# weigert/SoilMachine

Measured on AMD Instinct MI355X. Metric: particle-steps/s, higher is better.
Workload: dtype f64

## Files before the change

include/soilmx.h:

```cpp
#ifndef SOILMX_H
#define SOILMX_H
#include <stdint.h>

#ifdef __cplusplus
extern "C" {
#endif

typedef struct smx_ctx smx_ctx;

typedef struct smx_soil {
  uint32_t transports, erodes, cascades, abrades;
  float density, porosity, solubility, equrate, friction, erosionrate, maxdiff, settling, suspension, abrasion;
} smx_soil;

typedef struct smx_layer {
  uint32_t type;
  float min, bias, scale, octaves, lacunarity, gain, frequency;
} smx_layer;

enum { SMX_ENGINE_SERIAL = 0,
       SMX_ENGINE_SPECULATIVE = 1,
       SMX_ENGINE_BATCHED = 2,
       SMX_ENGINE_RELAXED = 3       };

// ... 159 lines not shown
int smx_fill_vertex_cut(smx_ctx* ctx, const float* colors4, int32_t ncolors, int32_t mode, double cut, int32_t x, int32_t y, void* out_vertex44);
int smx_heights_bilinear(smx_ctx* ctx, const float* pos2, int32_t n, double* out);

int smx_digest(smx_ctx* ctx, double* sumh, uint64_t* nsec, uint64_t* typehash);
int smx_switches(char* buf, uint64_t cap, uint64_t* needed);
int smx_get_counters_sized(smx_ctx* ctx, smx_counters* out, uint64_t struct_size);
int smx_get_timing_sized(smx_ctx* ctx, smx_timing* out, uint64_t struct_size);
int smx_get_counters(smx_ctx* ctx, smx_counters* out);
int smx_get_timing(smx_ctx* ctx, smx_timing* out);
int smx_timing_reset(smx_ctx* ctx);
int smx_set_engine(smx_ctx* ctx, int32_t engine);
int smx_set_spec_limits(smx_ctx* ctx, uint32_t particles_per_subphase, uint32_t nested_slots);
int smx_set_batch_dilate(smx_ctx* ctx, int32_t tiles);
int smx_set_relax_wind(smx_ctx* ctx, uint32_t min_running, int32_t steps_per_epoch);
int smx_set_relax_launch(smx_ctx* ctx, int32_t persistent, int32_t tail_at);
int smx_set_grid_interleave(smx_ctx* ctx, int32_t k);
int smx_set_water_generations(smx_ctx* ctx, int32_t k);
int smx_get_water_generations(smx_ctx* ctx, int32_t* k);
int smx_set_water_stagger(smx_ctx* ctx, int32_t gap_epochs);
int smx_get_water_stagger(smx_ctx* ctx, int32_t* gap_epochs);
int smx_set_batch_strips(smx_ctx* ctx, int32_t nstrips, int32_t inset, int32_t seam_halfwidth);
int smx_d_set_own(smx_ctx* ctx, int32_t own_x0, int32_t own_x1);
int smx_d_gen_begin(smx_ctx* ctx, int32_t wind, uint32_t nslots, const void* children, uint32_t* contains_out);
int smx_d_gen_spawn(smx_ctx* ctx, const uint32_t* contains, uint32_t* nlive_local);
int smx_d_next_phase(smx_ctx* ctx);
int smx_d_chunk(smx_ctx* ctx, uint32_t nlive_global, uint32_t* nlive_local);
int smx_d_gen_end(smx_ctx* ctx, void* children_out, uint32_t cap, uint32_t* n);
int smx_d_pack_columns(smx_ctx* ctx, int32_t x0, int32_t x1, void* buf, uint64_t cap, uint64_t* bytes);
int smx_d_unpack_columns(smx_ctx* ctx, const void* buf, uint64_t bytes);
int smx_d_pack_particles(smx_ctx* ctx, int32_t x0, int32_t x1, void* buf, uint64_t cap, uint64_t* bytes);
// ... 41 lines not shown
```

soilmachine_amd/capi.py:

```python
from __future__ import annotations

import ctypes as C
import os

import numpy as np

_HERE = os.path.dirname(os.path.abspath(__file__))
LIB_PATH = os.path.join(_HERE, "libsoilmx.so")

ENGINE_SERIAL = 0
ENGINE_SPECULATIVE = 1
ENGINE_BATCHED = 2
ENGINE_RELAXED = 3


class Config(C.Structure):
    _fields_ = [("dimx", C.c_int32), ("dimy", C.c_int32), ("scale", C.c_int32), ("device", C.c_int32),
                ("pool_capacity", C.c_uint64), ("engine", C.c_int32), ("reserved", C.c_int32)]


class Counters(C.Structure):
    _fields_ = [(n, C.c_uint64) for n in (
        "steps_water_top", "steps_water_all", "steps_wind", "nested_particles", "floods", "cascade_calls",
        "cascade_transfers", "wcascade_calls", "grid_active_cells", "rand_calls", "pool_free", "pool_overflow",
# ... 85 lines not shown
LAKE_DRY = 0xFFFFFFFF
LAKE_BORDER, LAKE_VOLUME_UNRELIABLE = 1, 2
DRAIN_NONE = 0xFFFFFFFF
BASIN_LAKE, BASIN_BORDER = 1, 2

PLANE_HEIGHT, PLANE_WATER, PLANE_WFREQ, PLANE_WINDFREQ = 0, 1, 2, 3
PLANES = {"height": PLANE_HEIGHT, "water": PLANE_WATER, "wfreq": PLANE_WFREQ, "windfreq": PLANE_WINDFREQ}


SYMBOLS = [
    "smx_create", "smx_create_strip", "smx_destroy", "smx_last_error", "smx_set_soils", "smx_set_scale", "smx_srand", "smx_rand", "smx_rand_advance", "smx_get_rand_state", "smx_set_rand_state",
    "smx_initialize", "smx_import_columns", "smx_import_frequency", "smx_num_sections", "smx_export_columns",
    "smx_read_frequency", "smx_read_heights", "smx_read_surface", "smx_tick_water", "smx_grid_pass", "smx_tick_wind",
    "smx_map_frequency", "smx_reset_frequency", "smx_tick", "smx_sync", "smx_add", "smx_remove",
    "smx_particle_cascade", "smx_water_cascade", "smx_seep", "smx_top", "smx_normals", "smx_heights_bilinear", "smx_fill_vertices", "smx_fill_vertices_cut", "smx_fill_vertex_cut",
    "smx_digest", "smx_save", "smx_load", "smx_get_counters", "smx_get_timing", "smx_get_counters_sized", "smx_get_timing_sized", "smx_timing_reset", "smx_set_engine", "smx_set_spec_limits", "smx_stream", "smx_set_batch_dilate", "smx_get_batch_stats", "smx_set_batch_strips", "smx_set_relax_wind", "smx_set_relax_launch", "smx_set_grid_interleave", "smx_set_water_generations", "smx_get_water_generations", "smx_set_water_stagger", "smx_get_water_stagger", "smx_strips_rccl_unique_id", "smx_strips_attach_rccl", "smx_strips_attach", "smx_strips_detach", "smx_strips_tick", "smx_strips_stats", "smx_strips_sync_stats", "smx_strips_selfcheck",
    "smx_d_set_own", "smx_d_gen_begin", "smx_d_gen_spawn", "smx_d_next_phase", "smx_d_chunk", "smx_d_gen_end", "smx_d_pack_columns",
    "smx_d_unpack_columns", "smx_d_pack_particles", "smx_d_unpack_particles", "smx_d_grid_begin", "smx_d_grid_sweep_cols",
    "smx_lbm_create", "smx_lbm_destroy", "smx_lbm_last_error", "smx_lbm_set_boundary", "smx_lbm_boundary_from_map", "smx_lbm_initialize",
    "smx_lbm_step", "smx_lbm_read", "smx_lbm_write_f", "smx_lbm_move", "smx_lbm_get_timing",
    "smx_ensemble_create", "smx_ensemble_destroy", "smx_ensemble_last_error", "smx_ensemble_add", "smx_ensemble_remove", "smx_ensemble_size",
    "smx_ensemble_tick", "smx_ensemble_sync", "smx_ensemble_get_timing", "smx_ensemble_timing_reset",
    "smx_ensemble_figures", "smx_ensemble_plane_stats", "smx_copy_state", "smx_ensemble_fork",
    "smx_lakes", "smx_ensemble_lakes", "smx_drainage", "smx_ensemble_drainage",
    "smx_soil_totals", "smx_ensemble_soil_totals", "smx_soil_thickness", "smx_cores",
    "smx_switches",
]

ENSEMBLE_MAX_MEMBERS = 4096

_lib = None
# ... 50 lines not shown
    L.smx_get_counters.argtypes = [vp, C.POINTER(Counters)]
    L.smx_get_timing.argtypes = [vp, C.POINTER(Timing)]
    L.smx_get_counters_sized.argtypes = [vp, C.POINTER(Counters), u64]
    L.smx_get_timing_sized.argtypes = [vp, C.POINTER(Timing), u64]
    L.smx_timing_reset.argtypes = [vp]
    L.smx_set_engine.argtypes = [vp, i32]
    L.smx_set_water_generations.argtypes = [vp, i32]
    L.smx_get_water_generations.argtypes = [vp, C.POINTER(i32)]
    L.smx_set_water_stagger.argtypes = [vp, i32]
    L.smx_get_water_stagger.argtypes = [vp, C.POINTER(i32)]
    L.smx_set_spec_limits.argtypes = [vp, C.c_uint32, C.c_uint32]
    L.smx_set_batch_dilate.argtypes = [vp, i32]
    L.smx_set_batch_strips.argtypes = [vp, i32, i32, i32]
    L.smx_set_relax_wind.argtypes = [vp, u32, i32]
    L.smx_set_relax_launch.argtypes = [vp, i32, i32]
    L.smx_create_strip.argtypes = [C.POINTER(Config), i32, i32, C.POINTER(vp)]
    L.smx_strips_rccl_unique_id.argtypes = [vp]
    L.smx_strips_attach_rccl.argtypes = [vp, vp, i32, i32, i32, i32]
    L.smx_strips_attach.argtypes = [vp, C.POINTER(Transport), i32, i32, i32, i32]
    L.smx_strips_detach.argtypes = [vp]
    L.smx_strips_tick.argtypes = [vp, i32, i32, i32, i32]
    L.smx_strips_stats.argtypes = [vp] + [C.POINTER(u64)] * 5
    L.smx_strips_sync_stats.argtypes = [vp] + [C.POINTER(u64)] * 2
    L.smx_strips_selfcheck.argtypes = [vp, u32, u32, u32]
    L.smx_d_set_own.argtypes = [vp, i32, i32]
    L.smx_d_gen_begin.argtypes = [vp, i32, u32, vp, vp]
    L.smx_d_gen_spawn.argtypes = [vp, vp, C.POINTER(u32)]
    L.smx_d_next_phase.argtypes = [vp]
    L.smx_d_chunk.argtypes = [vp, u32, C.POINTER(u32)]
    L.smx_d_gen_end.argtypes = [vp, vp, u32, C.POINTER(u32)]
# ... 70 lines not shown
```

soilmachine_amd/csrc/soil_relax.h:

```cpp
#pragma once
#include "soil_batch.h"

namespace smx {

constexpr uint32_t R_TRACK = 1, R_ERODE = 2, R_DEPOSIT = 4, R_WINDFREQ = 8, R_LIFT = 16;

#ifdef SMX_HOSTSIM
SMX_D uint32_t relax_append(uint32_t* counter, bool want) { return want ? SMX_A_ADD(counter, 1u) : NIL; }
#else
SMX_D uint32_t relax_append(uint32_t* counter, bool want) {
  const unsigned long long m = __ballot(want);
  if (!want) return NIL;
  const int leader = __ffsll((long long)m) - 1, lane = (int)(threadIdx.x & 63u);
  uint32_t base = 0u;
  if (lane == leader) base = atomicAdd(counter, (uint32_t)__popcll(m));
  base = (uint32_t)__shfl((int)base, leader);
  return base + (uint32_t)__popcll(m & ((1ull << lane) - 1ull));
}
#endif
SMX_D uint32_t relax_colour(const DevState& s, uint32_t c) {
  const uint32_t x = c / (uint32_t)s.dimy, y = c - x * (uint32_t)s.dimy;
  return (x % 3u) * 3u + (y % 3u);
}
SMX_D void relax_push(const DevState& s, const BatchShared& bs, uint32_t e, const RReq& r, uint32_t epoch) {
// ... 5 lines not shown
  if (flag) { if (k < bs.flag_cap) bs.flagl[par][k] = r.casc; else SMX_A_ADD(&bs.ctrl[BC_LIST_LOST], 1u); }
  (void)s;
}
SMX_D void relax_flood_later(const BatchShared& bs, uint32_t slot, uint32_t parity, bool want = true) {
  const uint32_t k = relax_append(&bs.ctrl[BC_NFLOOD + parity], want);
  if (want) { if (k < bs.list_cap) bs.flist[parity][k] = slot; else SMX_A_ADD(&bs.ctrl[BC_LIST_LOST], 1u); }
}
SMX_D void relax_reset_lists(const BatchShared& bs, uint32_t par) {
  bs.ctrl[BC_NFLOOD + par] = 0u; bs.ctrl[BC_NFLAG + par] = 0u; bs.ctrl[BC_NRUN + par] = 0u;
  for (uint32_t q = 0; q < 9u; q++) bs.ctrl[BC_NCASC + 9u * par + q] = 0u;
}
constexpr unsigned long long RELAX_FLOOD_SHARE = 64ull;
SMX_D bool relax_floods_due(const BatchShared& bs, uint32_t epoch, uint32_t nflood, uint32_t nrun) {
  return bs.strips.n > 1 || (epoch & 3u) == 3u || (unsigned long long)nflood * RELAX_FLOOD_SHARE >= (unsigned long long)nrun;
}
template <class P>
SMX_D void relax_filter(Sim<P>& sim, const BatchShared& bs, uint32_t c, bool valid, uint32_t epoch) {
  const DevState& s = sim.s;
  bool need = false; uint32_t col = 0u;
  if (valid) {
    const int x = (int)(c / (uint32_t)s.dimy), y = (int)(c - (uint32_t)x * (uint32_t)s.dimy);
    Blk b;
    sim.template load_block<2>(x, y, b);
    need = sim.cascade_precheck(b);
    if (!need) sim.n_casc++;
    else {
      bool alone = true;
      const int xa = x - 2 < s.x_lo ? s.x_lo : x - 2, xb = x + 2 >= s.x_hi ? s.x_hi - 1 : x + 2;
      const int ya = y - 2 < 0 ? 0 : y - 2, yb = y + 2 >= s.dimy ? s.dimy - 1 : y + 2;
      for (int xx = xa; xx <= xb; xx++)
        for (int yy = ya; yy <= yb; yy++)
          if ((xx != x || yy != y) && bs.cflag[(size_t)xx * (size_t)s.dimy + (size_t)yy] == bs.rtag) alone = false;
      if (alone) { sim.cascade_blk(x, y, b); need = false; }
    }
    col = (uint32_t)((x % 3) * 3 + (y % 3));
  }
  const uint32_t par = epoch & 1u;
#pragma unroll 1
  for (uint32_t q = 0; q < 9u; q++) {
    const bool mine = need && col == q;
    const uint32_t k = relax_append(&bs.ctrl[BC_NCASC + 9u * par + q], mine);
    if (mine) { if (k < bs.clist_cap) bs.clist[par][(size_t)q * bs.clist_cap + k] = c; else SMX_A_ADD(&bs.ctrl[BC_LIST_LOST], 1u); }
    if (mine && k < bs.clist_cap && bs.cstate) bs.cstate[c] = 2u * bs.rtag;
  }
}

template <class P>
// ... 177 lines not shown
```

soilmachine_amd/csrc/soilmx.hip:

```cpp
#include <hip/hip_runtime.h>
#include <stdint.h>
#include <stdio.h>
#include <string.h>
#include <stdlib.h>
#include <sys/stat.h>
#include <dlfcn.h>
#include <string>
#include <vector>

#include "../../include/soilmx.h"
#ifdef SMX_PROF_FLOOD
__device__ unsigned long long g_sect[32];
#endif
#include "soil_core.h"
#include "soil_serial.h"
#include "soil_spec.h"
#include <type_traits>
#include <chrono>
#include "soil_coop.h"
#include "soil_noise.h"
#include "soil_batch.h"
#include "soil_relax.h"
#include "soil_devmem.h"
#include "soil_lbm.h"
// ... 498 lines not shown
  }
  if (i >= nlive) return;
  BatchPolicy pol(s, bs);
  Sim<BatchPolicy> sim(s, sh, pol);
  relax_apply_slot(sim, bs, bs.live[i]);
  sim.flush_counters(); pol.finish(s);
}
__device__ __forceinline__ void relax_commit_cascade_counters(const DevState& s, unsigned long long nc, unsigned long long nt) {
  for (int off = 32; off > 0; off >>= 1) { nc += (unsigned long long)__shfl_down((long long)nc, off); nt += (unsigned long long)__shfl_down((long long)nt, off); }
  if ((threadIdx.x & 63u) == 0) { if (nc) atomicAdd(&s.ctr[C_CASCADE_CALLS], nc); if (nt) atomicAdd(&s.ctr[C_CASCADE_TRANSFERS], nt); }
}
__device__ __forceinline__ void relax_commit_flood_steps(const DevState& s, unsigned long long n) {
  for (int off = 32; off > 0; off >>= 1) n += (unsigned long long)__shfl_down((long long)n, off);
  if ((threadIdx.x & 63u) == 0 && n) atomicAdd(&s.ctr[C_FLOOD_NESTED_STEPS], n);
}
__global__ void __launch_bounds__(64) k_relax_filter(DevState s, BatchShared bs, uint32_t epoch) {
  const uint32_t par = epoch & 1u;
  uint32_t n = bs.ctrl[BC_NFLAG + par];
  if (n > bs.flag_cap) n = bs.flag_cap;
  if (blockIdx.x * 64u >= n) return;
  SMX_LOAD_SOILS(sh)
  const uint32_t i = blockIdx.x * 64u + threadIdx.x;
  BatchPolicy pol(s, bs);
  Sim<BatchPolicy> sim(s, sh, pol);
  relax_filter(sim, bs, i < n ? bs.flagl[par][i] : 0u, i < n, epoch);
  sim.flush_counters(); pol.finish(s);
  relax_commit_cascade_counters(s, pol.a_casc, pol.a_tr);
}
__global__ void __launch_bounds__(64) k_relax_cascade(DevState s, BatchShared bs, uint32_t epoch, uint32_t colour) {
  const uint32_t par = epoch & 1u;
  uint32_t n = bs.ctrl[BC_NCASC + 9u * par + colour];
  if (n > bs.clist_cap) n = bs.clist_cap;
  if (blockIdx.x * 64u >= n) return;
  SMX_LOAD_SOILS(sh)
  unsigned long long nc = 0, nt = 0;
  for (uint32_t i = blockIdx.x * 64u + threadIdx.x; i < n; i += gridDim.x * 64u) {
    BatchPolicy pol(s, bs);
    Sim<BatchPolicy> sim(s, sh, pol);
    relax_cascade(sim, bs.clist[par][(size_t)colour * bs.clist_cap + i]);
    sim.flush_counters(); pol.finish(s);
    nc += pol.a_casc; nt += pol.a_tr;
  }
  relax_commit_cascade_counters(s, nc, nt);
}
static uint32_t spin_budget(uint32_t dflt) { static const long long v = env_int("SMX_SPIN_BUDGET"); return v >= 0 ? (uint32_t)v : dflt; }
__device__ __forceinline__ bool spin_wait_while(const uint32_t* f, uint32_t busy, uint32_t* stalled, uint32_t budget, uint32_t sleep_a, uint32_t naps) {
  uint32_t spins = 0;
  while (__hip_atomic_load(f, __ATOMIC_RELAXED, __HIP_MEMORY_SCOPE_AGENT) == busy) {
    if (sleep_a == 2u) __builtin_amdgcn_s_sleep(2); else __builtin_amdgcn_s_sleep(8);
    for (uint32_t r = 0; r < naps; r++) __builtin_amdgcn_s_sleep(127);
    if (++spins > budget) { __hip_atomic_store(stalled, 1u, __ATOMIC_RELAXED, __HIP_MEMORY_SCOPE_AGENT); return false; }
    if ((spins & 1023u) == 0u && __hip_atomic_load(stalled, __ATOMIC_RELAXED, __HIP_MEMORY_SCOPE_AGENT)) return false;
  }
  return true;
}
__global__ void __launch_bounds__(64) k_relax_cascade_flow(DevState s, BatchShared bs, uint32_t epoch, uint32_t budget) {
  const uint32_t par = epoch & 1u;
  uint32_t cnt[9], total = 0;
#pragma unroll
  for (uint32_t q = 0; q < 9u; q++) { uint32_t n = bs.ctrl[BC_NCASC + 9u * par + q]; if (n > bs.clist_cap) n = bs.clist_cap; cnt[q] = n; total += n; }
  if (total == 0u) return;
  SMX_LOAD_SOILS(sh)
  __shared__ uint32_t s_i;
  unsigned long long nc = 0, nt = 0;
  const uint32_t pending = 2u * bs.rtag;
  bool live = true;
  while (true) {
    if (threadIdx.x == 0) s_i = atomicAdd(&bs.ctrl[BC_CASC_CURSOR], 1u);
    __syncthreads();
    uint32_t i = s_i;
    __syncthreads();
    if (i >= total) break;
    if (threadIdx.x == 0) {
      uint32_t q = 0;
#pragma unroll
      for (uint32_t k = 0; k < 9u; k++) { if (q == k && i >= cnt[k]) { i -= cnt[k]; q = k + 1u; } }
      const uint32_t c = bs.clist[par][(size_t)q * bs.clist_cap + i];
      const int x = (int)(c / (uint32_t)s.dimy), y = (int)(c - (uint32_t)x * (uint32_t)s.dimy);
      const int xa = x - 2 < s.x_lo ? s.x_lo : x - 2, xb = x + 2 >= s.x_hi ? s.x_hi - 1 : x + 2;
      const int ya = y - 2 < 0 ? 0 : y - 2, yb = y + 2 >= s.dimy ? s.dimy - 1 : y + 2;
      for (int xx = xa; xx <= xb; xx++)
        for (int yy = ya; yy <= yb; yy++) {
          if ((uint32_t)((xx % 3) * 3 + (yy % 3)) >= q) continue;
          uint32_t* f = &bs.cstate[(size_t)xx * (size_t)s.dimy + (size_t)yy];
          if (live && !spin_wait_while(f, pending, &bs.ctrl[BC_STALLED], budget, 2u, 0u)) live = false;
        }
      __atomic_thread_fence(__ATOMIC_ACQUIRE);
      BatchPolicy pol(s, bs);
      Sim<BatchPolicy> sim(s, sh, pol);
      relax_cascade(sim, c);
      sim.flush_counters(); pol.finish(s);
      nc += pol.a_casc; nt += pol.a_tr;
      __hip_atomic_store(&bs.cstate[c], pending + 1u, __ATOMIC_RELEASE, __HIP_MEMORY_SCOPE_AGENT);
    }
  }
  if (threadIdx.x == 0) { if (nc) atomicAdd(&s.ctr[C_CASCADE_CALLS], nc); if (nt) atomicAdd(&s.ctr[C_CASCADE_TRANSFERS], nt); }
}
__device__ unsigned long long g_flood_prof[72];
__global__ void __launch_bounds__(64) k_relax_floods(DevState s, BatchShared bs, uint32_t epoch, uint32_t prof) {
  const uint32_t par = epoch & 1u;
  uint32_t n = bs.ctrl[BC_NFLOOD + par];
  if (n > bs.list_cap) n = bs.list_cap;
  uint32_t lpw = (n + gridDim.x - 1u) / gridDim.x;
  if (lpw > 64u) lpw = 64u;
  if (blockIdx.x * lpw >= n) return;
  SMX_LOAD_SOILS(sh)
  const uint32_t i = blockIdx.x * lpw + threadIdx.x;
  const bool act = threadIdx.x < lpw && i < n;
  bool again = false; uint32_t slot = 0u;
  if (!relax_floods_due(bs, epoch, n, bs.ctrl[BC_NRUN + par])) {
    if (act) slot = bs.flist[par][i];
// ... 777 lines not shown
  bool batch_wind_buf = false;
  uint32_t* d_draws = nullptr; uint32_t* h_draws = nullptr; uint32_t draws_cap = 0;
  BChild* d_kids = nullptr; uint32_t kids_cap = 0;
  unsigned long long* d_skeys[2] = {nullptr, nullptr}; uint32_t* d_sidx[2] = {nullptr, nullptr}; void* d_stemp = nullptr; size_t stemp_bytes = 0; uint32_t sort_cap = 0;
  uint32_t* h_bctrl = nullptr;
  int batch_dilate = 0;
  uint32_t relax_wind_min = 0xFFFFFFFFu;
  int relax_wind_steps = 4;
  int relax_water_steps = 1;
  uint32_t relax_tag = 0;
  struct GridBar* d_gbar = nullptr;
  int mega_blocks = 0;
  bool mega_off = false;
  int relax_persistent = -1, relax_tail_at = -1;
  uint32_t flood_launch_no = 0;
  uint32_t relax_cap = 0;
  int strips_n = 1, strips_a = 16, strips_b = 48;
  int own_x0 = 0, own_x1 = -1;
  bool d_wind = false, d_first = true; uint32_t d_nslots = 0, d_epoch = 0, d_chunk = 0;
  uint32_t* d_contains = nullptr; uint32_t contains_cap = 0;
  uint8_t* d_xdata = nullptr; uint32_t* d_xoffs = nullptr; XCursor* d_xcur = nullptr;
  unsigned long long xdata_cap = 0; uint32_t xoffs_cap = 0;
  uint8_t* d_rdata = nullptr; uint32_t* d_roffs = nullptr; uint8_t* d_xpart = nullptr; uint8_t* d_rpart = nullptr; unsigned long long xpart_cap = 0;
  struct StripState* strip = nullptr;
  uint32_t* d_tdone = nullptr; uint32_t* d_tpend[2] = {nullptr, nullptr}; uint32_t* d_tcount = nullptr; uint32_t* h_tcount = nullptr; void* d_tsort = nullptr; size_t tsort_bytes = 0; uint32_t tsort_cap = 0;
  uint64_t batch_epochs = 0, batch_generations = 0, batch_children_lost = 0, grid_passes = 0;
  ForkScratch fork;
  LakeScratch lakes;
  DrainScratch drain;
  StrataScratch strata;
// ... 222 lines not shown
int smx_get_water_stagger(smx_ctx* ctx, int32_t* gap_epochs) { if (!gap_epochs) return -2; *gap_epochs = ctx->water_stagger; return 0; }
int smx_set_water_generations(smx_ctx* ctx, int32_t k) {
  if (k < 1 || k > 64) { ctx->err = "smx_set_water_generations: 1..64"; return -2; }
  ctx->water_generations = k;
  return 0;
}
int smx_set_grid_interleave(smx_ctx* ctx, int32_t) {
  ctx->err = "smx_set_grid_interleave: removed in round 5 (nested particles run inside their parent's region; the grid pass has no interleave any more)";
  return -2;
}
int smx_set_relax_launch(smx_ctx* ctx, int32_t persistent, int32_t tail_at) {
  if (tail_at > 256) { ctx->err = "smx_set_relax_launch: the tail kernel holds at most 256 particles (one per thread of its workgroup)"; return -2; }
  ctx->relax_persistent = persistent < 0 ? -1 : (persistent ? 1 : 0); ctx->relax_tail_at = tail_at < 0 ? -1 : tail_at;
  return 0;
}
int smx_set_relax_wind(smx_ctx* ctx, uint32_t min_running, int32_t steps_per_epoch) {
  if (steps_per_epoch < 1 || steps_per_epoch > R_MAXSTEPS) { ctx->err = "smx_set_relax_wind: 1..8 steps per epoch"; return -2; }
  ctx->relax_wind_min = min_running; ctx->relax_wind_steps = steps_per_epoch;
  return 0;
}
int smx_set_batch_strips(smx_ctx* ctx, int32_t nstrips, int32_t inset, int32_t seam_halfwidth) {
  if (nstrips < 1 || nstrips > 8 || inset < 0 || seam_halfwidth - inset < 32) { ctx->err = "smx_set_batch_strips: 1..8 strips, seam_halfwidth - inset >= 32"; return -2; }
  if (nstrips > 1 && ctx->cfg.dimx / nstrips < 2 * seam_halfwidth + 16) { ctx->err = "smx_set_batch_strips: strips narrower than two seam zones"; return -2; }
  if (nstrips > 1 && !batch_strips_fit(ctx->batch_dilate, inset, seam_halfwidth)) {
    ctx->err = "smx_set_batch_strips: the reservations of the current margin (smx_set_batch_dilate) do not fit seam_halfwidth - inset"; return -2;
  }
  ctx->strips_n = nstrips; ctx->strips_a = inset; ctx->strips_b = seam_halfwidth;
  return 0;
}
int smx_get_batch_stats(smx_ctx* ctx, uint64_t* epochs, uint64_t* generations, uint64_t* children_lost) {
// ... 590 lines not shown
  BatchShared bs = ctx->bs;
  uint32_t tag0 = ctx->relax_tag + 1u;
  GridBar* bar = ctx->d_gbar;
  static const uint32_t dense_waves_env = (uint32_t)env_int("SMX_RELAX_MEGA_WAVES");
  uint32_t dense_waves = dense_waves_env ? dense_waves_env : (uint32_t)ctx->mega_blocks, flags = relax_mega_flags();
  void* args[] = {(void*)&ctx->d, (void*)&bs, (void*)&nlive, (void*)&epoch, (void*)&nepochs, (void*)&tag0, (void*)&bar, (void*)&dense_waves, (void*)&flags};
  PhaseTimer tk(ctx, PH_K_EPOCHS, nepochs);
  const hipError_t e = hipLaunchCooperativeKernel((const void*)k_relax_epochs, dim3((unsigned)ctx->mega_blocks), dim3(256), args, 0, st);
  if (e != hipSuccess) {
    (void)hipGetLastError();
    fprintf(stderr, "[soilmx] hipLaunchCooperativeKernel(k_relax_epochs, %d workgroups): %s -- the relaxed epochs run as per-phase launches\n", ctx->mega_blocks, hipGetErrorString(e));
    ctx->mega_off = true; return 1;
  }
  return 0;
}
static int run_chunk(smx_ctx* ctx, bool wind, uint32_t nlive_sched, uint32_t nlive, uint32_t nslots, bool first, bool relax_gen, uint32_t& epoch, uint32_t& chunk,
                     int* epochs_run) {
  hipStream_t st = ctx->stream;
  const BatchShared& bs = ctx->bs;
  static const int CHUNK = (int)std::max(1ll, env_int("SMX_BATCH_CHUNK"));
  BSched sc = batch_schedule(wind, nlive_sched, ctx->batch_dilate);
  {
    static const char* ew = env_str("SMX_BATCH_SCHED"); static const char* ed = env_str("SMX_BATCH_SCHED_WIND");
    const char* e = wind ? ed : ew; int a, d, k;
    if (e && sscanf(e, "%d,%d,%d", &a, &d, &k) == 3) { sc.tshift = a; sc.dilate = d; sc.maxsteps = k; }
    static const char* etw = env_str("SMX_BATCH_SCHED_TAIL"); static const char* etd = env_str("SMX_BATCH_SCHED_TAIL_WIND");
    const char* et = wind ? etd : etw;
    if (et) {
      const char* q = et; unsigned thr;
      while (q && sscanf(q, "%u:%d,%d,%d", &thr, &a, &d, &k) == 4) {
// ... 29 lines not shown
      if (nslots) hipLaunchKernelGGL(k_relax_rebuild_floods, dim3((nslots + 255u) / 256u), dim3(256), 0, st, bs, nslots, epoch & 1u);
    }
    if (nlive == 0) { epoch += (uint32_t)chunk_epochs; ctx->relax_tag += (uint32_t)chunk_epochs; }
    else if (tail) {
      PhaseTimer tk(ctx, PH_K_TAIL, (uint32_t)chunk_epochs);
      hipLaunchKernelGGL(k_relax_tail, dim3(1), dim3(256), 0, st, ctx->d, bs, nlive, epoch, (uint32_t)chunk_epochs, ctx->relax_tag + 1u);
      ctx->relax_tag += (uint32_t)chunk_epochs; epoch += (uint32_t)chunk_epochs;
    } else if (mega && relax_epochs_launch(ctx, nlive, epoch, (uint32_t)chunk_epochs) == 0) {
      ctx->relax_tag += (uint32_t)chunk_epochs; epoch += (uint32_t)chunk_epochs;
    } else {
      const uint32_t lpw = batch_lanes_per_wave(nlive);
      const unsigned nbl = (nlive + lpw - 1u) / lpw, nb64 = (nlive + 63u) / 64u;
      const unsigned ncb = (unsigned)(((size_t)nlive * (size_t)(wind ? ctx->bs.rstride : ctx->bs.rsteps) + 63u) / 64u);
      static const unsigned fb_min = (unsigned)env_int("SMX_RELAX_FLOOD_BLOCKS");
      const unsigned nfb = std::max(fb_min, (unsigned)((nslots + 63u) / 64u));
      for (int k = 0; k < chunk_epochs; k++, epoch++) {
        ctx->bs.rtag = ++ctx->relax_tag;
        {
          static const int sample = (int)std::max(0ll, env_int("SMX_STEP_EVENT_SAMPLE"));
          const bool timed = sample > 0 && (k % sample) == 0;
          if (wind) ctx->timing.launches_step_wind++; else ctx->timing.launches_step_water++;
          if (timed) { PhaseTimer tk(ctx, wind ? PH_K_WIND : PH_K_WATER, 1u); LAUNCH_WIND_WATER(wind, k_relax_step, dim3(nbl), dim3(64), st, ctx->d, bs, nlive, epoch, lpw); }
          else LAUNCH_WIND_WATER(wind, k_relax_step, dim3(nbl), dim3(64), st, ctx->d, bs, nlive, epoch, lpw);
        }
        hipLaunchKernelGGL(k_relax_apply, dim3(nb64), dim3(64), 0, st, ctx->d, bs, nlive, epoch);
        hipLaunchKernelGGL(k_relax_filter, dim3(ncb), dim3(64), 0, st, ctx->d, bs, epoch);
        static const unsigned casc_blocks = (unsigned)env_int("SMX_RELAX_CASC_BLOCKS");
        static const unsigned casc_flow = (unsigned)env_int("SMX_RELAX_CASC_FLOW");
        if (casc_flow && bs.cstate) hipLaunchKernelGGL(k_relax_cascade_flow, dim3(std::min(ncb, casc_flow)), dim3(64), 0, st, ctx->d, bs, epoch, spin_budget(1u << 24));
        else {
          const unsigned ncc = std::min(ncb, std::max(1u, casc_blocks));
          for (uint32_t col = 0; col < 9u; col++) hipLaunchKernelGGL(k_relax_cascade, dim3(ncc), dim3(64), 0, st, ctx->d, bs, epoch, col);
        }
        if (!wind) {
          ctx->timing.launches_floods_all++;
          const uint32_t fprof = flood_prof();
          if (ctx->flood_launch_no++ % 7u == 0u) { PhaseTimer tk(ctx, PH_K_FLOODS, 1u); hipLaunchKernelGGL(k_relax_floods, dim3(nfb), dim3(64), 0, st, ctx->d, bs, epoch, fprof); }
          else hipLaunchKernelGGL(k_relax_floods, dim3(nfb), dim3(64), 0, st, ctx->d, bs, epoch, fprof);
        }
      }
    }
  } else if (nlive) {
    PhaseTimer tk(ctx, wind ? PH_K_WIND : PH_K_WATER, (uint32_t)CHUNK);
    if (wind) ctx->timing.launches_step_wind += (uint64_t)CHUNK; else ctx->timing.launches_step_water += (uint64_t)CHUNK;
    const uint32_t lpw = batch_lanes_per_wave(nlive);
    const unsigned nbl = (nlive + lpw - 1u) / lpw;
    static const uint32_t occ2_above = (uint32_t)env_int("SMX_BATCH_OCC2_ABOVE");
// ... 1549 lines not shown
```

soilmachine_amd/machine.py:

```python
from __future__ import annotations

import ctypes as C

import numpy as np

from . import capi
from .snapshot import Snapshot
from .soilfile import SoilConfig, soils_array, layers_array


class SoilmxError(RuntimeError):
    pass


POOLSIZE = 10_000_000


def default_pool(dimx: int, dimy: int) -> int:
    return max(POOLSIZE, 4 * int(dimx) * int(dimy))


class Layermap:

    def __init__(self, cfg: SoilConfig, dimx: int | None = None, dimy: int | None = None, *, seed: int = 0,
# ... 215 lines not shown

    def counters(self) -> dict:
        c = capi.Counters()
        self._chk(self.L.smx_get_counters_sized(self.h, C.byref(c), C.sizeof(c)))
        return c.as_dict()

    def set_batch_dilate(self, tiles: int):
        self._chk(self.L.smx_set_batch_dilate(self.h, int(tiles)))

    def set_relax_wind(self, min_running: int = 0xFFFFFFFF, steps_per_epoch: int = 4):
        self._chk(self.L.smx_set_relax_wind(self.h, int(min_running), int(steps_per_epoch)))

    def set_relax_launch(self, persistent: int = -1, tail_at: int = -1):
        self._chk(self.L.smx_set_relax_launch(self.h, int(persistent), int(tail_at)))

    def set_water_generations(self, k: int):
        self._chk(self.L.smx_set_water_generations(self.h, int(k)))

    def set_water_stagger(self, gap_epochs: int):
        self._chk(self.L.smx_set_water_stagger(self.h, int(gap_epochs)))

    def water_stagger(self) -> int:
        g = C.c_int32()
        self._chk(self.L.smx_get_water_stagger(self.h, C.byref(g)))
        return int(g.value)

    def water_generations(self) -> int:
        k = C.c_int32()
        self._chk(self.L.smx_get_water_generations(self.h, C.byref(k)))
        return int(k.value)
# ... 54 lines not shown
```

Baseline: 63.95 million.

## Fuse relax filter and cascade into one settle kernel with per-cell waits

Adds a k_relax_settle kernel that runs the cascade precheck, the crowding test and the colour-ordered cascades inside one launch. Uncrowded cells cascade at once, and crowded cells wait on their neighbours' cstate flags through wavefront-wide spin polling, which replaces the separate filter and flow-cascade launches. The filter kernel now packs a configurable number of cells per wavefront, and the flow cascade waits on neighbours in parallel across lanes with an explicit release publish. The risks are spin-wait stalls or deadlock when the grid is not fully resident, and lower lane utilisation in the filter.

```diff
diff --git a/include/soilmx.h b/include/soilmx.h
--- a/include/soilmx.h
+++ b/include/soilmx.h
@@ -197,6 +197,8 @@
 int smx_set_batch_dilate(smx_ctx* ctx, int32_t tiles);
 int smx_set_relax_wind(smx_ctx* ctx, uint32_t min_running, int32_t steps_per_epoch);
 int smx_set_relax_launch(smx_ctx* ctx, int32_t persistent, int32_t tail_at);
+int smx_set_relax_settle(smx_ctx* ctx, int32_t mode, int32_t max_waves, int32_t lanes);
+int smx_get_relax_settle(smx_ctx* ctx, uint64_t* crowded_cells, uint64_t* epochs_fused, uint64_t* epochs_split);
 int smx_set_grid_interleave(smx_ctx* ctx, int32_t k);
 int smx_set_water_generations(smx_ctx* ctx, int32_t k);
 int smx_get_water_generations(smx_ctx* ctx, int32_t* k);
diff --git a/soilmachine_amd/capi.py b/soilmachine_amd/capi.py
--- a/soilmachine_amd/capi.py
+++ b/soilmachine_amd/capi.py
@@ -123,7 +123,7 @@
     "smx_read_frequency", "smx_read_heights", "smx_read_surface", "smx_tick_water", "smx_grid_pass", "smx_tick_wind",
     "smx_map_frequency", "smx_reset_frequency", "smx_tick", "smx_sync", "smx_add", "smx_remove",
     "smx_particle_cascade", "smx_water_cascade", "smx_seep", "smx_top", "smx_normals", "smx_heights_bilinear", "smx_fill_vertices", "smx_fill_vertices_cut", "smx_fill_vertex_cut",
-    "smx_digest", "smx_save", "smx_load", "smx_get_counters", "smx_get_timing", "smx_get_counters_sized", "smx_get_timing_sized", "smx_timing_reset", "smx_set_engine", "smx_set_spec_limits", "smx_stream", "smx_set_batch_dilate", "smx_get_batch_stats", "smx_set_batch_strips", "smx_set_relax_wind", "smx_set_relax_launch", "smx_set_grid_interleave", "smx_set_water_generations", "smx_get_water_generations", "smx_set_water_stagger", "smx_get_water_stagger", "smx_strips_rccl_unique_id", "smx_strips_attach_rccl", "smx_strips_attach", "smx_strips_detach", "smx_strips_tick", "smx_strips_stats", "smx_strips_sync_stats", "smx_strips_selfcheck",
+    "smx_digest", "smx_save", "smx_load", "smx_get_counters", "smx_get_timing", "smx_get_counters_sized", "smx_get_timing_sized", "smx_timing_reset", "smx_set_engine", "smx_set_spec_limits", "smx_stream", "smx_set_batch_dilate", "smx_get_batch_stats", "smx_set_batch_strips", "smx_set_relax_wind", "smx_set_relax_launch", "smx_set_relax_settle", "smx_get_relax_settle", "smx_set_grid_interleave", "smx_set_water_generations", "smx_get_water_generations", "smx_set_water_stagger", "smx_get_water_stagger", "smx_strips_rccl_unique_id", "smx_strips_attach_rccl", "smx_strips_attach", "smx_strips_detach", "smx_strips_tick", "smx_strips_stats", "smx_strips_sync_stats", "smx_strips_selfcheck",
     "smx_d_set_own", "smx_d_gen_begin", "smx_d_gen_spawn", "smx_d_next_phase", "smx_d_chunk", "smx_d_gen_end", "smx_d_pack_columns",
     "smx_d_unpack_columns", "smx_d_pack_particles", "smx_d_unpack_particles", "smx_d_grid_begin", "smx_d_grid_sweep_cols",
     "smx_lbm_create", "smx_lbm_destroy", "smx_lbm_last_error", "smx_lbm_set_boundary", "smx_lbm_boundary_from_map", "smx_lbm_initialize",
@@ -204,6 +204,8 @@
     L.smx_set_batch_strips.argtypes = [vp, i32, i32, i32]
     L.smx_set_relax_wind.argtypes = [vp, u32, i32]
     L.smx_set_relax_launch.argtypes = [vp, i32, i32]
+    L.smx_set_relax_settle.argtypes = [vp, i32, i32, i32]
+    L.smx_get_relax_settle.argtypes = [vp, C.POINTER(u64), C.POINTER(u64), C.POINTER(u64)]
     L.smx_create_strip.argtypes = [C.POINTER(Config), i32, i32, C.POINTER(vp)]
     L.smx_strips_rccl_unique_id.argtypes = [vp]
     L.smx_strips_attach_rccl.argtypes = [vp, vp, i32, i32, i32, i32]
diff --git a/soilmachine_amd/csrc/soil_relax.h b/soilmachine_amd/csrc/soil_relax.h
--- a/soilmachine_amd/csrc/soil_relax.h
+++ b/soilmachine_amd/csrc/soil_relax.h
@@ -43,7 +43,23 @@
 SMX_D bool relax_floods_due(const BatchShared& bs, uint32_t epoch, uint32_t nflood, uint32_t nrun) {
   return bs.strips.n > 1 || (epoch & 3u) == 3u || (unsigned long long)nflood * RELAX_FLOOD_SHARE >= (unsigned long long)nrun;
 }
-template <class P>
+SMX_D bool relax_crowded(const DevState& s, const BatchShared& bs, int x, int y) {
+  uint32_t f[25];
+#pragma unroll
+  for (int k = 0; k < 25; k++) {
+    const int xx = x + k / 5 - 2, yy = y + k % 5 - 2;
+    const int xc = xx < s.x_lo ? s.x_lo : (xx >= s.x_hi ? s.x_hi - 1 : xx), yc = yy < 0 ? 0 : (yy >= s.dimy ? s.dimy - 1 : yy);
+    f[k] = k == 12 ? 0u : bs.cflag[(size_t)xc * (size_t)s.dimy + (size_t)yc];
+  }
+  bool any = false;
+#pragma unroll
+  for (int k = 0; k < 25; k++) {
+    const int xx = x + k / 5 - 2, yy = y + k % 5 - 2;
+    if (k != 12 && xx >= s.x_lo && xx < s.x_hi && yy >= 0 && yy < s.dimy && f[k] == bs.rtag) any = true;
+  }
+  return any;
+}
+template <class P, bool BATCHED = false>
 SMX_D void relax_filter(Sim<P>& sim, const BatchShared& bs, uint32_t c, bool valid, uint32_t epoch) {
   const DevState& s = sim.s;
   bool need = false; uint32_t col = 0u;
@@ -55,11 +71,14 @@
     if (!need) sim.n_casc++;
     else {
       bool alone = true;
-      const int xa = x - 2 < s.x_lo ? s.x_lo : x - 2, xb = x + 2 >= s.x_hi ? s.x_hi - 1 : x + 2;
-      const int ya = y - 2 < 0 ? 0 : y - 2, yb = y + 2 >= s.dimy ? s.dimy - 1 : y + 2;
-      for (int xx = xa; xx <= xb; xx++)
-        for (int yy = ya; yy <= yb; yy++)
-          if ((xx != x || yy != y) && bs.cflag[(size_t)xx * (size_t)s.dimy + (size_t)yy] == bs.rtag) alone = false;
+      if constexpr (BATCHED) alone = !relax_crowded(s, bs, x, y);
+      else {
+        const int xa = x - 2 < s.x_lo ? s.x_lo : x - 2, xb = x + 2 >= s.x_hi ? s.x_hi - 1 : x + 2;
+        const int ya = y - 2 < 0 ? 0 : y - 2, yb = y + 2 >= s.dimy ? s.dimy - 1 : y + 2;
+        for (int xx = xa; xx <= xb; xx++)
+          for (int yy = ya; yy <= yb; yy++)
+            if ((xx != x || yy != y) && bs.cflag[(size_t)xx * (size_t)s.dimy + (size_t)yy] == bs.rtag) alone = false;
+      }
       if (alone) { sim.cascade_blk(x, y, b); need = false; }
     }
     col = (uint32_t)((x % 3) * 3 + (y % 3));
diff --git a/soilmachine_amd/csrc/soilmx.hip b/soilmachine_amd/csrc/soilmx.hip
--- a/soilmachine_amd/csrc/soilmx.hip
+++ b/soilmachine_amd/csrc/soilmx.hip
@@ -536,16 +536,17 @@
   for (int off = 32; off > 0; off >>= 1) n += (unsigned long long)__shfl_down((long long)n, off);
   if ((threadIdx.x & 63u) == 0 && n) atomicAdd(&s.ctr[C_FLOOD_NESTED_STEPS], n);
 }
-__global__ void __launch_bounds__(64) k_relax_filter(DevState s, BatchShared bs, uint32_t epoch) {
+__global__ void __launch_bounds__(64) k_relax_filter(DevState s, BatchShared bs, uint32_t epoch, uint32_t lpw) {
   const uint32_t par = epoch & 1u;
   uint32_t n = bs.ctrl[BC_NFLAG + par];
   if (n > bs.flag_cap) n = bs.flag_cap;
-  if (blockIdx.x * 64u >= n) return;
+  if (blockIdx.x * lpw >= n) return;
   SMX_LOAD_SOILS(sh)
-  const uint32_t i = blockIdx.x * 64u + threadIdx.x;
+  const uint32_t i = blockIdx.x * lpw + threadIdx.x;
+  const bool valid = threadIdx.x < lpw && i < n;
   BatchPolicy pol(s, bs);
   Sim<BatchPolicy> sim(s, sh, pol);
-  relax_filter(sim, bs, i < n ? bs.flagl[par][i] : 0u, i < n, epoch);
+  relax_filter<BatchPolicy, true>(sim, bs, valid ? bs.flagl[par][i] : 0u, valid, epoch);
   sim.flush_counters(); pol.finish(s);
   relax_commit_cascade_counters(s, pol.a_casc, pol.a_tr);
 }
@@ -576,6 +577,34 @@
   }
   return true;
 }
+__device__ __forceinline__ void relax_publish(uint32_t* f, uint32_t v) {
+  __builtin_amdgcn_fence(__ATOMIC_RELEASE, "agent");
+  asm volatile("s_waitcnt vmcnt(0)" ::: "memory");
+  __hip_atomic_store(f, v, __ATOMIC_RELAXED, __HIP_MEMORY_SCOPE_AGENT);
+}
+template <bool SETTLE>
+__device__ __forceinline__ bool relax_wait_block(const DevState& s, const BatchShared& bs, uint32_t c, uint32_t q, uint32_t budget) {
+  const uint32_t lane = threadIdx.x & 63u, t2 = 2u * bs.rtag;
+  const int x = (int)(c / (uint32_t)s.dimy), y = (int)(c - (uint32_t)x * (uint32_t)s.dimy);
+  const int xx = x + (int)(lane / 5u) - 2, yy = y + (int)(lane % 5u) - 2;
+  const bool inr = lane < 25u && lane != 12u && xx >= s.x_lo && xx < s.x_hi && yy >= 0 && yy < s.dimy;
+  const size_t ci = inr ? (size_t)xx * (size_t)s.dimy + (size_t)yy : (size_t)c;
+  const bool earlier = inr && (uint32_t)((xx % 3) * 3 + (yy % 3)) < q;
+  const bool watch = SETTLE ? (inr && bs.cflag[ci] == bs.rtag) : earlier;
+  uint32_t* stalled = &bs.ctrl[BC_STALLED];
+  uint32_t spins = 0;
+  while (true) {
+    bool ok = true;
+    if (watch) {
+      const uint32_t st = __hip_atomic_load(&bs.cstate[ci], __ATOMIC_RELAXED, __HIP_MEMORY_SCOPE_AGENT);
+      ok = SETTLE ? (st >= t2 && (!earlier || st == t2 + 1u)) : st != t2;
+    }
+    if (__ballot(!ok) == 0ull) return true;
+    __builtin_amdgcn_s_sleep(2);
+    if (++spins > budget) { if (lane == 0u) __hip_atomic_store(stalled, 1u, __ATOMIC_RELAXED, __HIP_MEMORY_SCOPE_AGENT); return false; }
+    if ((spins & 1023u) == 0u && __hip_atomic_load(stalled, __ATOMIC_RELAXED, __HIP_MEMORY_SCOPE_AGENT)) return false;
+  }
+}
 __global__ void __launch_bounds__(64) k_relax_cascade_flow(DevState s, BatchShared bs, uint32_t epoch, uint32_t budget) {
   const uint32_t par = epoch & 1u;
   uint32_t cnt[9], total = 0;
@@ -583,40 +612,82 @@
   for (uint32_t q = 0; q < 9u; q++) { uint32_t n = bs.ctrl[BC_NCASC + 9u * par + q]; if (n > bs.clist_cap) n = bs.clist_cap; cnt[q] = n; total += n; }
   if (total == 0u) return;
   SMX_LOAD_SOILS(sh)
-  __shared__ uint32_t s_i;
+  __shared__ uint32_t s_i, s_c, s_q;
   unsigned long long nc = 0, nt = 0;
   const uint32_t pending = 2u * bs.rtag;
   bool live = true;
   while (true) {
-    if (threadIdx.x == 0) s_i = atomicAdd(&bs.ctrl[BC_CASC_CURSOR], 1u);
+    if (threadIdx.x == 0) {
+      uint32_t i = atomicAdd(&bs.ctrl[BC_CASC_CURSOR], 1u), q = 0;
+      s_i = i;
+      if (i < total) {
+#pragma unroll
+        for (uint32_t k = 0; k < 9u; k++) { if (q == k && i >= cnt[k]) { i -= cnt[k]; q = k + 1u; } }
+        s_c = bs.clist[par][(size_t)q * bs.clist_cap + i]; s_q = q;
+      }
+    }
     __syncthreads();
-    uint32_t i = s_i;
+    const uint32_t i = s_i, c = s_c, q = s_q;
     __syncthreads();
     if (i >= total) break;
+    if (live && !relax_wait_block<false>(s, bs, c, q, budget)) live = false;
     if (threadIdx.x == 0) {
-      uint32_t q = 0;
-#pragma unroll
-      for (uint32_t k = 0; k < 9u; k++) { if (q == k && i >= cnt[k]) { i -= cnt[k]; q = k + 1u; } }
-      const uint32_t c = bs.clist[par][(size_t)q * bs.clist_cap + i];
-      const int x = (int)(c / (uint32_t)s.dimy), y = (int)(c - (uint32_t)x * (uint32_t)s.dimy);
-      const int xa = x - 2 < s.x_lo ? s.x_lo : x - 2, xb = x + 2 >= s.x_hi ? s.x_hi - 1 : x + 2;
-      const int ya = y - 2 < 0 ? 0 : y - 2, yb = y + 2 >= s.dimy ? s.dimy - 1 : y + 2;
-      for (int xx = xa; xx <= xb; xx++)
-        for (int yy = ya; yy <= yb; yy++) {
-          if ((uint32_t)((xx % 3) * 3 + (yy % 3)) >= q) continue;
-          uint32_t* f = &bs.cstate[(size_t)xx * (size_t)s.dimy + (size_t)yy];
-          if (live && !spin_wait_while(f, pending, &bs.ctrl[BC_STALLED], budget, 2u, 0u)) live = false;
-        }
       __atomic_thread_fence(__ATOMIC_ACQUIRE);
       BatchPolicy pol(s, bs);
       Sim<BatchPolicy> sim(s, sh, pol);
       relax_cascade(sim, c);
       sim.flush_counters(); pol.finish(s);
       nc += pol.a_casc; nt += pol.a_tr;
-      __hip_atomic_store(&bs.cstate[c], pending + 1u, __ATOMIC_RELEASE, __HIP_MEMORY_SCOPE_AGENT);
+      relax_publish(&bs.cstate[c], pending + 1u);
     }
   }
   if (threadIdx.x == 0) { if (nc) atomicAdd(&s.ctr[C_CASCADE_CALLS], nc); if (nt) atomicAdd(&s.ctr[C_CASCADE_TRANSFERS], nt); }
+}
+__global__ void __launch_bounds__(64) k_relax_settle(DevState s, BatchShared bs, uint32_t epoch, uint32_t lpw, uint32_t budget, unsigned long long* ncrowded) {
+  const uint32_t par = epoch & 1u;
+  uint32_t n = bs.ctrl[BC_NFLAG + par];
+  if (n > bs.flag_cap) n = bs.flag_cap;
+  if (blockIdx.x * lpw >= n) return;
+  SMX_LOAD_SOILS(sh)
+  const uint32_t lane = threadIdx.x, i = blockIdx.x * lpw + lane, t2 = 2u * bs.rtag;
+  const bool valid = lane < lpw && i < n;
+  const uint32_t c = valid ? bs.flagl[par][i] : 0u;
+  BatchPolicy pol(s, bs);
+  Sim<BatchPolicy> sim(s, sh, pol);
+  uint32_t kind = 0u, col = 0u;
+  if (valid) {
+    const int x = (int)(c / (uint32_t)s.dimy), y = (int)(c - (uint32_t)x * (uint32_t)s.dimy);
+    Blk b;
+    sim.template load_block<2>(x, y, b);
+    if (!sim.cascade_precheck(b)) sim.n_casc++;
+    else kind = relax_crowded(s, bs, x, y) ? 2u : 1u;
+    col = (uint32_t)((x % 3) * 3 + (y % 3));
+    relax_publish(&bs.cstate[c], kind ? t2 : t2 + 1u);
+  }
+  const unsigned long long crowd = __ballot(kind == 2u);
+  if (lane == 0u && crowd) atomicAdd(ncrowded, (unsigned long long)__popcll(crowd));
+  bool live = true;
+  for (int q = -1; q < 9; q++) {
+    unsigned long long m = __ballot(q < 0 ? kind == 1u : (kind == 2u && col == (uint32_t)q));
+    while (m) {
+      bool mine;
+      if (q < 0) { mine = kind == 1u; m = 0ull; }
+      else {
+        const int owner = __ffsll((long long)m) - 1;
+        m &= m - 1ull;
+        const uint32_t cc = (uint32_t)__shfl((int)c, owner);
+        if (live && !relax_wait_block<true>(s, bs, cc, (uint32_t)q, budget)) live = false;
+        __builtin_amdgcn_fence(__ATOMIC_ACQUIRE, "agent");
+        mine = (int)lane == owner;
+      }
+      if (mine) {
+        relax_cascade(sim, c);
+        relax_publish(&bs.cstate[c], t2 + 1u);
+      }
+    }
+  }
+  sim.flush_counters(); pol.finish(s);
+  relax_commit_cascade_counters(s, pol.a_casc, pol.a_tr);
 }
 __device__ unsigned long long g_flood_prof[72];
 __global__ void __launch_bounds__(64) k_relax_floods(DevState s, BatchShared bs, uint32_t epoch, uint32_t prof) {
@@ -1424,6 +1495,11 @@
   bool mega_off = false;
   int relax_persistent = -1, relax_tail_at = -1;
   uint32_t flood_launch_no = 0;
+  int relax_settle = -1;
+  int settle_max_waves = 0, settle_lanes = 0;
+  int settle_resident = 0;
+  unsigned long long* d_settle_crowded = nullptr;
+  uint64_t settle_epochs_fused = 0, settle_epochs_split = 0;
   uint32_t relax_cap = 0;
   int strips_n = 1, strips_a = 16, strips_b = 48;
   int own_x0 = 0, own_x1 = -1;
@@ -1676,6 +1752,22 @@
   ctx->relax_persistent = persistent < 0 ? -1 : (persistent ? 1 : 0); ctx->relax_tail_at = tail_at < 0 ? -1 : tail_at;
   return 0;
 }
+int smx_set_relax_settle(smx_ctx* ctx, int32_t mode, int32_t max_waves, int32_t lanes) {
+  if (mode > 1 || lanes > 64) { ctx->err = "smx_set_relax_settle: mode -1, 0 or 1; at most 64 cells per wavefront"; return -2; }
+  ctx->relax_settle = mode < 0 ? -1 : mode; ctx->settle_max_waves = max_waves < 0 ? 0 : max_waves; ctx->settle_lanes = lanes < 0 ? 0 : lanes;
+  return 0;
+}
+int smx_get_relax_settle(smx_ctx* ctx, uint64_t* crowded_cells, uint64_t* epochs_fused, uint64_t* epochs_split) {
+  unsigned long long nc = 0;
+  if (ctx->d_settle_crowded) {
+    HIPCHK(ctx, hipMemcpyAsync(&nc, ctx->d_settle_crowded, sizeof(nc), hipMemcpyDeviceToHost, ctx->stream));
+    HIPCHK(ctx, hipStreamSynchronize(ctx->stream));
+  }
+  if (crowded_cells) *crowded_cells = nc;
+  if (epochs_fused) *epochs_fused = ctx->settle_epochs_fused;
+  if (epochs_split) *epochs_split = ctx->settle_epochs_split;
+  return 0;
+}
 int smx_set_relax_wind(smx_ctx* ctx, uint32_t min_running, int32_t steps_per_epoch) {
   if (steps_per_epoch < 1 || steps_per_epoch > R_MAXSTEPS) { ctx->err = "smx_set_relax_wind: 1..8 steps per epoch"; return -2; }
   ctx->relax_wind_min = min_running; ctx->relax_wind_steps = steps_per_epoch;
@@ -2296,6 +2388,29 @@
   }
   return 0;
 }
+constexpr uint32_t RELAX_SETTLE_LANES = 8;
+static uint32_t relax_settle_lanes(size_t worst, size_t waves, uint32_t forced) {
+  uint32_t l = forced ? forced : RELAX_SETTLE_LANES;
+  while (l < 64u && (worst + l - 1u) / l > waves) l = std::min(64u, l * 2u);
+  return (worst + l - 1u) / l > waves ? 0u : l;
+}
+constexpr int RELAX_SETTLE_DEFAULT = 1;
+static uint32_t relax_settle_plan(smx_ctx* ctx, size_t worst) {
+  if (!ctx->settle_resident) {
+    int dev = 0, ncu = 0, per_cu = 0;
+    hipGetDevice(&dev);
+    hipDeviceGetAttribute(&ncu, hipDeviceAttributeMultiprocessorCount, dev);
+    if (hipOccupancyMaxActiveBlocksPerMultiprocessor(&per_cu, k_relax_settle, 64, 0) != hipSuccess) { (void)hipGetLastError(); per_cu = 0; }
+    ctx->settle_resident = ncu * per_cu > 0 ? ncu * per_cu : -1;
+  }
+  if (ctx->settle_resident < 0) return 0u;
+  if (!ctx->d_settle_crowded) {
+    if (ctx->mem.dev(ctx->d_settle_crowded, 1) != hipSuccess) { (void)hipGetLastError(); ctx->settle_resident = -1; return 0u; }
+    hipMemsetAsync(ctx->d_settle_crowded, 0, sizeof(unsigned long long), ctx->stream);
+  }
+  const size_t waves = ctx->settle_max_waves > 0 ? std::min<size_t>((size_t)ctx->settle_max_waves, (size_t)ctx->settle_resident) : (size_t)ctx->settle_resident;
+  return relax_settle_lanes(worst, waves, (uint32_t)ctx->settle_lanes);
+}
 static int run_chunk(smx_ctx* ctx, bool wind, uint32_t nlive_sched, uint32_t nlive, uint32_t nslots, bool first, bool relax_gen, uint32_t& epoch, uint32_t& chunk,
                      int* epochs_run) {
   hipStream_t st = ctx->stream;
@@ -2355,6 +2470,13 @@
       const unsigned ncb = (unsigned)(((size_t)nlive * (size_t)(wind ? ctx->bs.rstride : ctx->bs.rsteps) + 63u) / 64u);
       static const unsigned fb_min = (unsigned)env_int("SMX_RELAX_FLOOD_BLOCKS");
       const unsigned nfb = std::max(fb_min, (unsigned)((nslots + 63u) / 64u));
+      static const unsigned casc_blocks = (unsigned)env_int("SMX_RELAX_CASC_BLOCKS");
+      static const unsigned casc_flow = (unsigned)env_int("SMX_RELAX_CASC_FLOW");
+      const size_t worst = (size_t)nlive * (size_t)(wind ? ctx->bs.rstride : ctx->bs.rsteps);
+      const bool settle_on = (ctx->relax_settle >= 0 ? ctx->relax_settle : RELAX_SETTLE_DEFAULT) == 1 && !strips && casc_flow && bs.cstate;
+      const uint32_t settle_lpw = settle_on ? relax_settle_plan(ctx, worst) : 0u;
+      uint32_t filter_lpw = relax_settle_lanes(worst, 4096u, (uint32_t)ctx->settle_lanes);
+      if (!filter_lpw) filter_lpw = 64u;
       for (int k = 0; k < chunk_epochs; k++, epoch++) {
         ctx->bs.rtag = ++ctx->relax_tag;
         {
@@ -2365,13 +2487,17 @@
           else LAUNCH_WIND_WATER(wind, k_relax_step, dim3(nbl), dim3(64), st, ctx->d, bs, nlive, epoch, lpw);
         }
         hipLaunchKernelGGL(k_relax_apply, dim3(nb64), dim3(64), 0, st, ctx->d, bs, nlive, epoch);
-        hipLaunchKernelGGL(k_relax_filter, dim3(ncb), dim3(64), 0, st, ctx->d, bs, epoch);
-        static const unsigned casc_blocks = (unsigned)env_int("SMX_RELAX_CASC_BLOCKS");
-        static const unsigned casc_flow = (unsigned)env_int("SMX_RELAX_CASC_FLOW");
-        if (casc_flow && bs.cstate) hipLaunchKernelGGL(k_relax_cascade_flow, dim3(std::min(ncb, casc_flow)), dim3(64), 0, st, ctx->d, bs, epoch, spin_budget(1u << 24));
-        else {
-          const unsigned ncc = std::min(ncb, std::max(1u, casc_blocks));
-          for (uint32_t col = 0; col < 9u; col++) hipLaunchKernelGGL(k_relax_cascade, dim3(ncc), dim3(64), 0, st, ctx->d, bs, epoch, col);
+        if (settle_lpw) {
+          ctx->settle_epochs_fused++;
+          hipLaunchKernelGGL(k_relax_settle, dim3((unsigned)((worst + settle_lpw - 1u) / settle_lpw)), dim3(64), 0, st, ctx->d, bs, epoch, settle_lpw, spin_budget(1u << 24), ctx->d_settle_crowded);
+        } else {
+          ctx->settle_epochs_split++;
+          hipLaunchKernelGGL(k_relax_filter, dim3((unsigned)((worst + filter_lpw - 1u) / filter_lpw)), dim3(64), 0, st, ctx->d, bs, epoch, filter_lpw);
+          if (casc_flow && bs.cstate) hipLaunchKernelGGL(k_relax_cascade_flow, dim3(std::min(ncb, casc_flow)), dim3(64), 0, st, ctx->d, bs, epoch, spin_budget(1u << 24));
+          else {
+            const unsigned ncc = std::min(ncb, std::max(1u, casc_blocks));
+            for (uint32_t col = 0; col < 9u; col++) hipLaunchKernelGGL(k_relax_cascade, dim3(ncc), dim3(64), 0, st, ctx->d, bs, epoch, col);
+          }
         }
         if (!wind) {
           ctx->timing.launches_floods_all++;
diff --git a/soilmachine_amd/machine.py b/soilmachine_amd/machine.py
--- a/soilmachine_amd/machine.py
+++ b/soilmachine_amd/machine.py
@@ -253,6 +253,14 @@
     def set_relax_launch(self, persistent: int = -1, tail_at: int = -1):
         self._chk(self.L.smx_set_relax_launch(self.h, int(persistent), int(tail_at)))
 
+    def set_relax_settle(self, mode: int = -1, max_waves: int = 0, lanes: int = 0):
+        self._chk(self.L.smx_set_relax_settle(self.h, int(mode), int(max_waves), int(lanes)))
+
+    def relax_settle_stats(self) -> dict:
+        c, f, s = C.c_uint64(), C.c_uint64(), C.c_uint64()
+        self._chk(self.L.smx_get_relax_settle(self.h, C.byref(c), C.byref(f), C.byref(s)))
+        return {"crowded_cells": int(c.value), "epochs_fused": int(f.value), "epochs_split": int(s.value)}
+
     def set_water_generations(self, k: int):
         self._chk(self.L.smx_set_water_generations(self.h, int(k)))
 
```

Result: faster. 67.99 million, median of 6 (+6.3%).
